# dusk-network/schnorr

Measured on AMD Instinct MI355X. Metric: Schnorr verifies/sec (single + double) at batch=2^20; 1/2/4/8 MI355X, higher is better.
Workload: dtype u32x9 (29-bit limbs, u64 accumulate); 1 GPU; 2^20 single-signature batch verify per GPU (BASELINE configs[1]); `value` is this figure, `double` / `vargen` / `mixed` ride along with --full; batch_per_gpu=1048576, parallelism=dp1, collective=none

## Files before the change

schnorr_amd/csrc/dsv_host.h:

```cpp
#pragma once
#include <hip/hip_runtime.h>

#include <atomic>
#include <chrono>
#include <condition_variable>
#include <cstdarg>
#include <cstdio>
#include <cstring>
#include <functional>
#include <initializer_list>
#include <mutex>
#include <string>
#include <thread>
#include <type_traits>
#include <vector>

#include <errno.h>
#include <sys/random.h>

#include "../../include/dsv.h"
#include "launch.h"
#include "rlc.h"
#include "host_sync.h"

namespace dsvh {

using namespace dsv;
typedef uint32_t u32;

extern thread_local std::string g_err;
int fail(int code, const char* fmt, ...);
#define HIP_TRY(expr)                                                                         \
  do {                                                                                        \
    hipError_t e_ = (expr);                                                                   \
    if (e_ != hipSuccess)                                                                     \
      return fail(DSV_ERR_HIP, "%s failed: %s (%s:%d)", #expr, hipGetErrorString(e_), __FILE__, \
                  __LINE__);                                                                  \
  } while (0)

constexpr int kPipeSlots = 8;
constexpr int kMaxDevices = 16;
constexpr int kSplitLanes = 8;

struct SplitLane {
  hipStream_t owner = nullptr;
  bool made = false;
  hipStream_t stream[2] = {nullptr, nullptr};
  hipStream_t side = nullptr;
  hipEvent_t fork = nullptr, join[2] = {nullptr, nullptr}, side_join = nullptr;
};

struct PipeSlot {
  hipEvent_t ev_in = nullptr;
  hipEvent_t ev_pre = nullptr;
  hipEvent_t ev_lane[2] = {nullptr, nullptr};
  hipEvent_t ev_done = nullptr;
  uint8_t* prep = nullptr;
  size_t prep_bytes = 0;
  uint8_t* stage = nullptr;
  size_t bytes = 0;
  uint8_t* host = nullptr;
  size_t host_bytes = 0;
};
struct Pipe {
  PipeSlot slot[kPipeSlots];
  CopyPool copiers;
};

struct Context {
  std::atomic<bool> ready{false};
  int device = -1;
  std::string pci_bdf;
  int numa_node = -1;
  std::vector<int> numa_cpus;
  bool split = true;
  bool fuse_double = true;
  bool quad = true;
  bool small_overlap = true;
  u32* table[2] = {nullptr, nullptr};
  u32* ts_cancel = nullptr;
  uint8_t* ts_hash = nullptr;
  std::mutex mu;
  uint8_t* stage = nullptr;
  size_t stage_bytes = 0;
  std::mutex lane_mu;
  SplitLane lanes[kSplitLanes];
  PipeSync pipe_sync;
  Pipe pipes[kPipes];
  std::mutex enq_mu;
  bool pipe_made = false;
  bool pipe_failed = false;
  hipStream_t pipe_in = nullptr, pipe_out = nullptr, pipe_lane[2] = {nullptr, nullptr}, pipe_pre = nullptr;
  hipStream_t pipe_small = nullptr;
  uint8_t* pipe_work[3] = {};
  size_t pipe_work_bytes[3] = {};
  uint64_t pipe_parts = 0;
  long lane_load[2] = {0, 0};
  bool prep_stream = false;
  PlanParams plan;
  int pipe_slots = 0;
  int norm_per_lane = 0, norm_block = 0;
  struct RlcHostArena {
    std::mutex mu;
    uint8_t* dev = nullptr;
    size_t bytes = 0;
    hipStream_t stream = nullptr;
    hipEvent_t ev[2] = {nullptr, nullptr};
  } rlc_arenas[2];
  std::mutex rlc_pinned_mu;
  u32* rlc_pinned = nullptr;
  std::atomic<u32> rlc_slot{0};
};
extern Context g_ctx[kMaxDevices];
extern std::mutex g_init_mu;
extern std::atomic<int> g_primary;
extern thread_local int t_device;
extern std::mutex g_jobs_mu;
extern std::condition_variable g_jobs_cv;
extern int g_jobs;

struct DeviceGuard {
  int prev = -1;
  bool switched = false;
  hipError_t err = hipSuccess;
  explicit DeviceGuard(int device) {
    err = hipGetDevice(&prev);
    if (err == hipSuccess && prev != device) {
      err = hipSetDevice(device);
      switched = err == hipSuccess;
    }
  }
  ~DeviceGuard() {
    if (switched) (void)hipSetDevice(prev);
  }
};
#define DSV_ON_DEVICE(ctx)                     \
  DeviceGuard guard_((ctx).device);            \
  if (guard_.err != hipSuccess)                \
  return fail(DSV_ERR_HIP, "cannot select device %d: %s", (ctx).device, hipGetErrorString(guard_.err))

int ensure_stage(Context& ctx, size_t bytes);
void destroy_pipe_streams(Context& ctx);
int ensure_pipe_streams(Context& ctx);
int ensure_pipe_work(Context& ctx, int lane, size_t bytes);
int ensure_pipe_slot(PipeSlot& sl, size_t dev_bytes, size_t host_bytes, size_t prep_bytes);
int check_n(size_t n);
int host_context(Context*& out);
int device_context(const void* ptr, Context*& out);
void release_context(Context& ctx);
void keysets_release_device(int device);

struct Workspace {
  uint8_t* c;
  uint8_t* valid;
  u32* tables;
};
constexpr int kTablesPerLane = 3;
inline size_t var_table_bytes(size_t n, int tables_per_lane) {
  return (size_t)verify_grid(n) * kVerifyBlock * kVarLaneWords * 4 * (size_t)tables_per_lane;
}
inline Workspace carve(void* ws, size_t n) {
  Workspace w;
  w.c = static_cast<uint8_t*>(ws);
  w.valid = w.c + align_up(n * 32, 256);
  w.tables = reinterpret_cast<u32*>(w.valid + align_up(n, 256));
  return w;
}

struct Stager {
  uint8_t* base;
  size_t off = 0;
  explicit Stager(uint8_t* b) : base(b) {}
  uint8_t* take(size_t bytes) {
    uint8_t* p = base + off;
    off += align_up(bytes, 256);
    return p;
  }
};

void launch_verify_fixed(const Context& ctx, bool accumulate, const void* u, const void* c,
                         const void* PK_uv, const void* R_uv, int which, const void* valid,
                         size_t n, void* ok, u32* tables, hipStream_t s, bool tables_ready = false,
                         const u32* gate = nullptr);
void launch_verify_fixed_double(const Context& ctx, const void* u, const void* c, const void* PK_uv,
                                const void* R_uv, const void* PKp_uv, const void* Rp_uv,
                                const void* valid, size_t n, void* ok, u32* tables, hipStream_t s,
                                bool tables_ready = false, const u32* gate = nullptr);


int acquire_lane(Context& ctx, hipStream_t user, SplitLane*& out);
template <class Part>
int run_split(Context& ctx, size_t n, void* workspace, hipStream_t user, Part part) {
  Workspace w = carve(workspace, n);
  if (!ctx.split || n < 2 * kSplitItems) {
    part((size_t)0, n, w, user);
    HIP_TRY(hipGetLastError());
    return DSV_OK;
  }
  SplitLane* lane = nullptr;
  if (int r = acquire_lane(ctx, user, lane)) return r;
  std::lock_guard<std::mutex> lk(ctx.lane_mu);
  HIP_TRY(hipEventRecord(lane->fork, user));
  const size_t tbl_words = var_table_bytes(kSplitItems, kTablesPerLane) / 4;
  for (int k = 0; k < 2; k++) HIP_TRY(hipStreamWaitEvent(lane->stream[k], lane->fork, 0));
  size_t off = 0;
  for (size_t p = 0; off < n; p++) {
    const size_t cnt = n - off < kSplitItems ? n - off : kSplitItems;
    const int k = (int)(p & 1);
    Workspace wp;
    wp.c = w.c + off * 32;
    wp.valid = w.valid + off;
    wp.tables = w.tables + (size_t)k * tbl_words;
    part(off, cnt, wp, lane->stream[k]);
    off += cnt;
  }
  HIP_TRY(hipGetLastError());
  for (int k = 0; k < 2; k++) {
    HIP_TRY(hipEventRecord(lane->join[k], lane->stream[k]));
    HIP_TRY(hipStreamWaitEvent(user, lane->join[k], 0));
  }
  return DSV_OK;
}

#define DSV_DEV_PROLOGUE(n, owner_ptr)              \
  if (int r_ = check_n(n)) return r_;               \
  if ((n) == 0) return DSV_OK;                      \
  Context* ctxp_ = nullptr;                         \
  if (int r_ = device_context(owner_ptr, ctxp_)) return r_; \
  Context& ctx = *ctxp_;                            \
  DSV_ON_DEVICE(ctx)


struct SchemeLayout {
  int points;
  size_t sig_bytes, pk_bytes;
  int R, Rp, PK, PKp, Gen;
  bool fixed;
};
constexpr SchemeLayout kSchemes[3] = {
    {2, 64, 32, 0, -1, 1, -1, -1, true},
    {4, 96, 64, 0, 1, 2, 3, -1, true},
    {3, 64, 64, 0, -1, 1, -1, 2, false},
};
inline const SchemeLayout& layout(int scheme) { return kSchemes[scheme]; }
struct Items {
  int scheme = 0;
  const uint8_t* u = nullptr;
  const uint8_t* pt[4] = {};
  const uint8_t* m = nullptr;
  Items at(size_t off, size_t pt_bytes = 64) const {
    Items r = *this;
    r.u = u + 32 * off;
    for (int k = 0; k < layout(scheme).points; k++) r.pt[k] = pt[k] ? pt[k] + pt_bytes * off : nullptr;
    r.m = m ? m + 32 * off : nullptr;
    return r;
  }
  const uint8_t* slot(int k) const { return k < 0 ? nullptr : pt[k]; }
  const uint8_t* R() const { return slot(layout(scheme).R); }
  const uint8_t* Rp() const { return slot(layout(scheme).Rp); }
  const uint8_t* PK() const { return slot(layout(scheme).PK); }
  const uint8_t* PKp() const { return slot(layout(scheme).PKp); }
  const uint8_t* Gen() const { return slot(layout(scheme).Gen); }
  bool any_null() const {
    bool r = !u || !m;
    for (int k = 0; k < layout(scheme).points; k++) r = r || !pt[k];
    return r;
  }
};
inline Items make_items(int scheme, const void* u, std::initializer_list<const void*> pts, const void* m) {
  Items in{scheme, static_cast<const uint8_t*>(u)};
  int k = 0;
  for (const void* p : pts) in.pt[k++] = static_cast<const uint8_t*>(p);
  in.m = static_cast<const uint8_t*>(m);
  return in;
}

extern thread_local bool t_pipeline_part;
extern thread_local size_t t_chunk_first;
void launch_hash(const Items& in, size_t n, uint8_t* c, uint8_t* valid, hipStream_t s, const uint8_t* valid_in = nullptr);
void launch_verify(const Context& ctx, const Items& in, const uint8_t* c, const uint8_t* valid, size_t n,
                   uint8_t* ok, u32* tables, hipStream_t s, bool prebuilt = false, const u32* gate = nullptr);
int verify_on(Context& ctx, const Items& in, size_t n, void* ok, void* workspace, hipStream_t stream,
              const uint8_t* valid_in = nullptr);
void normalize_on(int scheme, const uint8_t* const* in, uint8_t* const* out, size_t n, uint8_t* valid, u32* prefix,
                  hipStream_t s, const uint8_t* u_mont = nullptr, const uint8_t* m_mont = nullptr,
                  uint8_t* u_out = nullptr, uint8_t* m_out = nullptr, int per_lane = 0, int block = 0);
int decompress_on(Context& ctx, const void* in, size_t in_stride, size_t n, void* out_uv, void* ok,
                  int accumulate, hipStream_t stream);

struct RlcStaged {
  ChaChaKey key;
  size_t boundary;
};
int verify_rlc_on(Context& ctx, const Items& in, size_t n, void* ok, void* workspace, hipStream_t s, int window_bits,
                  u32* accepted_dev, bool and_into = false, bool have_challenges = false,
                  const uint8_t* valid_in = nullptr, const RlcStaged* staged = nullptr);
struct RlcVerdictTarget {
  u32* dev = nullptr;
  u32* slot = nullptr;
  int* out = nullptr;
};
int rlc_verdict_target(Context& ctx, int* accepted, RlcVerdictTarget& t);
int rlc_verdict_wait(const RlcVerdictTarget& t, hipStream_t s);
int rlc_clear_accepted(int* accepted);
int rlc_history(Context& ctx);
void carve_rlc_buffers(Stager& st, const RlcPlan& p, RlcBuffers& b);
size_t rlc_group_items(size_t n);
int rlc_split_groups(size_t cnt, int window_bits);
RlcPlan rlc_group_plan(int scheme, size_t cnt, int window_bits, int groups, bool keyed = false);
int check_rlc_bits(int window_bits);
int rlc_random_key(ChaChaKey& key);
int refuse_capture(hipStream_t s, const char* what);
void rlc_plan_words(const RlcPlan& p, size_t bytes, uint64_t* out);
int rlc_forced_groups();
u32* rlc_keyed_history(Context& ctx);

#define H2D(dst, src, bytes) HIP_TRY(hipMemcpyAsync((dst), (src), (bytes), hipMemcpyHostToDevice, 0))
#define D2H(dst, src, bytes) HIP_TRY(hipMemcpyAsync((dst), (src), (bytes), hipMemcpyDeviceToHost, 0))
#define DSV_HOST_PROLOGUE(n)                                  \
  if (int r_ = check_n(n)) return r_;                         \
  if ((n) == 0) return DSV_OK;                                \
  Context* ctxp_ = nullptr;                                   \
  if (int r_ = host_context(ctxp_)) return r_;                \
  Context& ctx = *ctxp_
#define DSV_HOST_LOCK()                                                                \
  std::lock_guard<std::mutex> lk(ctx.mu);                                              \
  if (!ctx.ready.load(std::memory_order_acquire))                                      \
    return fail(DSV_ERR_NOT_INITIALIZED, "device %d was shut down", ctx.device);       \
  DSV_ON_DEVICE(ctx)


constexpr size_t kExtItemBytes = 4 * 64 + 1 + 4 * kLimbs * 4 + 1;
constexpr size_t kMontItemBytes = kExtItemBytes + 64;
enum Form { kAffine, kExt, kMont };
inline size_t form_pt_bytes(int form) { return form == kAffine ? 64 : 96; }
int check_cols(int scheme, const dsv_column* cols, size_t n, const uint8_t* ok, int form);
int verify_host_cols(int scheme, int form, const dsv_column* cols, size_t n, uint8_t* ok, bool multi);

struct WireWs {
  uint8_t *u, *R, *Rp, *P0, *P1, *valid;
  Items items(int scheme, const void* m) const {
    const uint8_t* sig_pts[2] = {R, Rp};
    const uint8_t* pk_pts[2] = {P0, P1};
    const int ns = (int)(layout(scheme).sig_bytes / 32) - 1;
    Items in{scheme, u};
    for (int k = 0; k < layout(scheme).points; k++) in.pt[k] = k < ns ? sig_pts[k] : pk_pts[k - ns];
    in.m = static_cast<const uint8_t*>(m);
    return in;
  }
};
WireWs carve_wire(Stager& x, size_t n);
int decode_wire(Context& ctx, int scheme, const uint8_t* sig, const uint8_t* pk, size_t n, const Items& out,
                uint8_t* valid, hipStream_t st);
int verify_wire(Context& ctx, int scheme, const uint8_t* sig, const uint8_t* pk, const uint8_t* m,
                size_t n, uint8_t* ok);

}
```

schnorr_amd/csrc/k_verify.hip:

```cpp
#include "common.h"
#include "halfgcd.h"

namespace dsv {

template <int NCHAIN>
__global__ void __launch_bounds__(kVerifyBlock, kWavesVerify)
k_verify_fixed_half(const uint8_t* __restrict__ u, const uint8_t* __restrict__ c, ChainOperands op0,
                    ChainOperands op1, const uint8_t* __restrict__ valid, bool accumulate, size_t n,
                    uint8_t* __restrict__ ok, u32* __restrict__ var_tables, const u32* __restrict__ gate) {
  if (gate_says_done(gate)) return;
  u32* tbl = var_tables + ((size_t)blockIdx.x * kVerifyBlock + threadIdx.x) * kJointLaneWords;
#pragma unroll 1
  for (size_t base = (size_t)blockIdx.x * kVerifyBlock; base < n;
       base += (size_t)gridDim.x * kVerifyBlock) {
    const size_t i = base + threadIdx.x;
    if (i >= n) continue;
    bool good = accumulate ? (ok[i] != 0) : (valid[i] != 0);
    u32 ya[8], yb[8], w[8];
    bool b_neg;
    int top;
    {
      u32 cs[8], a[8], b[8];
      load_words8(cs, c, i);
      half_scalars(a, b, b_neg, cs);
      recode_signed2(ya, a);
      recode_signed2(yb, b);
      u32 nz[8];
#pragma unroll
      for (int k = 0; k < 8; k++) nz[k] = (ya[k] ^ 0x55555555u) | (yb[k] ^ 0x55555555u);
      top = top_digit2(nz);
      u32 us[8];
      load_words8(us, u, i);
      const bool u_ok = words_lt(us, kR32);
      good &= u_ok;
      if (!u_ok) us[7] &= 0x0fffffffu;
      fr_mul(w, b, us);
      if (b_neg) {
        const u32 zero[8] = {0, 0, 0, 0, 0, 0, 0, 0};
        u32 t[8];
        fr_sub(t, zero, w);
#pragma unroll
        for (int k = 0; k < 8; k++) w[k] = t[k];
      }
    }
#pragma unroll 1
    for (int h = 0; h < NCHAIN; h++) {
      const ChainOperands op = h ? op1 : op0;
      {
        Fe pku, pkv, ru, rv;
        good &= load_fq(pku, op.PK_uv, 2 * i);
        good &= load_fq(pkv, op.PK_uv, 2 * i + 1);
        good &= load_fq_signed(ru, op.R_uv, 2 * i, !b_neg);
        good &= load_fq(rv, op.R_uv, 2 * i + 1);
        build_joint_table(tbl, pku, pkv, ru, rv);
      }
      Ext acc = ext_from_niels(load_var_entry(tbl, joint_digit(ya, yb, top)));
      {
        RawNiels e = load_var_entry_raw(tbl, joint_digit(ya, yb, top > 0 ? top - 1 : 0));
#pragma unroll 1
        for (int k = top - 1; k >= 0; k--) {
          acc = ext_mul4(acc);
          const Niels cur = finish_var_entry(e);
          e = load_var_entry_raw(tbl, joint_digit(ya, yb, k > 0 ? k - 1 : 0));
          acc = ext_add_niels(acc, cur);
        }
      }
      good &= fixed_base_accumulate_is_identity(acc, w, op.table);
    }
    ok[i] = good ? 1 : 0;
  }
}

void launch_verify_half(int nchain, bool accumulate, const uint8_t* u, const uint8_t* c,
                        ChainOperands op0, ChainOperands op1, const uint8_t* valid, size_t n,
                        uint8_t* ok, uint32_t* var_tables, hipStream_t s, const uint32_t* gate) {
  const dim3 grid(verify_grid(n)), block(kVerifyBlock);
  if (nchain == 2)
    hipLaunchKernelGGL(k_verify_fixed_half<2>, grid, block, 0, s, u, c, op0, op1, valid, accumulate, n,
                       ok, var_tables, gate);
  else
    hipLaunchKernelGGL(k_verify_fixed_half<1>, grid, block, 0, s, u, c, op0, op1, valid, accumulate, n,
                       ok, var_tables, gate);
}

}
```

schnorr_amd/csrc/launch.h:

```cpp
#pragma once
#include <hip/hip_runtime.h>
#include <stddef.h>
#include <stdint.h>

namespace dsv {

constexpr int kLimbs = 9;

constexpr int kFixedBits = 16;
constexpr int kFixedWindows = (253 + kFixedBits - 1) / kFixedBits;
constexpr int kFixedEntries = (1 << (kFixedBits - 1)) + 1;
constexpr int kEntryWords = 4 * kLimbs;
constexpr size_t kTableBytes = (size_t)kFixedWindows * kFixedEntries * kEntryWords * 4;
static_assert(kFixedWindows * kFixedBits <= 288 && kFixedBits >= 4 && kFixedBits <= 16, "window");

constexpr int kVarEntries = 9;
constexpr int kVarEntryWords = 4 * kLimbs;
constexpr int kVarLaneWords = kVarEntries * kVarEntryWords;
constexpr int kVerifyBlock = 64;
constexpr unsigned kMaxVerifyGrid = 4096;
constexpr int kWavesVerify = 2, kWavesHash = 2;

constexpr int kQuadBlock = 256;
constexpr size_t kQuadMaxItems = (size_t)1 << 14;
constexpr size_t kVarHexMaxItems = (size_t)1 << 13;

constexpr int kSplitThreads = 256;
constexpr int kSplitPerThread = 16;
constexpr int kSplitTile = kSplitThreads * kSplitPerThread;

inline unsigned grid_for(size_t n, unsigned block = 256) { return (unsigned)((n + block - 1) / block); }
inline unsigned verify_grid(size_t n) {
  const unsigned g = grid_for(n, kVerifyBlock);
  return g < kMaxVerifyGrid ? g : kMaxVerifyGrid;
}

struct ChainOperands {
  const uint8_t* PK_uv;
  const uint8_t* R_uv;
  const uint32_t* table;
};
struct ChaChaKey {
  uint32_t w[8];
};

hipError_t hash_upload_constants();
void launch_challenge(bool dbl, const uint8_t* R_uv, const uint8_t* Rp_uv, const uint8_t* m, size_t n,
                      uint8_t* c, uint8_t* valid, hipStream_t s, const uint8_t* valid_in = nullptr);
inline __device__ bool gate_says_done(const uint32_t* gate) { return gate && gate[0] == 0u && gate[1] == 1u; }
void launch_verify_half(int nchain, bool accumulate, const uint8_t* u, const uint8_t* c,
                        ChainOperands op0, ChainOperands op1, const uint8_t* valid, size_t n,
                        uint8_t* ok, uint32_t* var_tables, hipStream_t s, const uint32_t* gate = nullptr);
void launch_verify_half_quad(int nchain, bool accumulate, bool tables_ready, const uint8_t* u,
                             const uint8_t* c, ChainOperands op0, ChainOperands op1,
                             const uint8_t* valid, size_t n, uint8_t* ok, uint32_t* var_tables,
                             hipStream_t s, const uint32_t* gate = nullptr);
void launch_prep_var_tables(const uint8_t* PK_uv, const uint8_t* R_uv, size_t n, uint32_t* var_tables,
                            hipStream_t s);
void launch_verify_var(const uint8_t* u, const uint8_t* c, const uint8_t* PK_uv, const uint8_t* Gen_uv,
                       const uint8_t* R_uv, const uint8_t* valid, size_t n, uint8_t* ok,
                       uint32_t* var_tables, hipStream_t s, const uint32_t* gate = nullptr);
void launch_debug_lattice3(const uint8_t* u, const uint8_t* c, size_t n, uint8_t* out, hipStream_t s);
void launch_debug_half_scalars(const uint8_t* c, size_t n, uint8_t* out, hipStream_t s);
void launch_var_base_points(const uint8_t* scalar, const uint8_t* P_uv, size_t n, uint8_t* out_uv,
                            uint32_t* var_tables, hipStream_t s);
void launch_build_fixed_table(uint32_t* table, int which, hipStream_t s);
void launch_fixed_base_points(const uint8_t* scalar, const uint32_t* table, size_t n, uint8_t* out_uv,
                              hipStream_t s);
struct NormalizeArgs {
  const uint8_t* in[4];
  uint8_t* out[4];
  const uint8_t* u_mont = nullptr;
  const uint8_t* m_mont = nullptr;
  uint8_t* u_out = nullptr;
  uint8_t* m_out = nullptr;
};
constexpr int kNormalizePerLane = 32;
inline size_t normalize_lanes(size_t n, int& per_lane, int want_per_lane = 0) {
  per_lane = n >= ((size_t)1 << 19) ? 16 : (n >= ((size_t)1 << 15) ? 8 : 1);
  if (want_per_lane > 0) per_lane = want_per_lane > kNormalizePerLane ? kNormalizePerLane : want_per_lane;
  return (n + per_lane - 1) / per_lane;
}
inline size_t normalize_prefix_bytes(size_t n, int npoints) {
  return (size_t)npoints * (n + kNormalizePerLane) * kLimbs * 4;
}
void launch_normalize_uvz(const NormalizeArgs& a, int npoints, size_t n, uint8_t* valid,
                          uint32_t* prefix, hipStream_t s, int want_per_lane = 0, int block = 0);
void launch_sign_finish(const uint8_t* r, const uint8_t* c, const uint8_t* sk, size_t n, uint8_t* u_out,
                        hipStream_t s);
void launch_decompress(const uint8_t* in, size_t in_stride, size_t n, uint8_t* out_uv, uint8_t* ok,
                       int accumulate, const uint32_t* ts_cancel, const uint8_t* ts_hash, hipStream_t s);
void launch_gather32(const uint8_t* in, size_t stride, size_t n, uint8_t* out, hipStream_t s);
void launch_stdrng_triples(ChaChaKey key, size_t first_item, size_t n, uint8_t* sk, uint8_t* m,
                           uint8_t* r, hipStream_t s);
void launch_stdrng_quads(ChaChaKey key, size_t first_item, size_t n, uint8_t* sk, uint8_t* g,
                         uint8_t* m, uint8_t* r, hipStream_t s);
void launch_debug_fq_mul(const uint8_t* a, const uint8_t* b, size_t n, uint8_t* out, hipStream_t s);
void launch_split_kinds(const uint8_t* kinds, size_t n, uint32_t* tile_counts, uint32_t* totals,
                        uint32_t* idx0, size_t cap0, uint32_t* idx1, size_t cap1, hipStream_t s);
void launch_gather_rows(const void* src, size_t src_rows, uint32_t row16, const uint32_t* idx,
                        size_t count, const uint32_t* limit, void* dst, hipStream_t s);
void launch_scatter_bytes(const uint8_t* src, const uint32_t* idx, size_t count, const uint32_t* limit,
                          uint8_t* dst, size_t dst_len, hipStream_t s);
void launch_mixed_check(const uint32_t* totals, uint32_t want0, uint32_t want1, uint8_t* ok, size_t n,
                        hipStream_t s);

}
```

Baseline: 85.98 million verifies/s.

## Sort verify lanes by top joint digit within larger blocks to cut divergence

The block grows to a configurable group of 256 threads. Each item's top recoded digit is computed first, then items are counting-sorted in shared memory by that digit, so lanes in a wave run similar ladder lengths and divergence in the variable-base loop drops. Item index, sign and top digit are packed into a meta word, and the scalar words are exchanged through LDS. This adds shared-memory traffic, three block barriers per iteration and a larger block under the same launch bounds, which could cost registers or occupancy. The var table sizing is updated to match the new grid.

```diff
diff --git a/schnorr_amd/csrc/dsv_host.h b/schnorr_amd/csrc/dsv_host.h
--- a/schnorr_amd/csrc/dsv_host.h
+++ b/schnorr_amd/csrc/dsv_host.h
@@ -157,7 +157,7 @@
 };
 constexpr int kTablesPerLane = 3;
 inline size_t var_table_bytes(size_t n, int tables_per_lane) {
-  return (size_t)verify_grid(n) * kVerifyBlock * kVarLaneWords * 4 * (size_t)tables_per_lane;
+  return (size_t)verify_group_grid(n) * kVerifyGroup * kVarLaneWords * 4 * (size_t)tables_per_lane;
 }
 inline Workspace carve(void* ws, size_t n) {
   Workspace w;
diff --git a/schnorr_amd/csrc/k_verify.hip b/schnorr_amd/csrc/k_verify.hip
--- a/schnorr_amd/csrc/k_verify.hip
+++ b/schnorr_amd/csrc/k_verify.hip
@@ -3,39 +3,80 @@
 
 namespace dsv {
 
+constexpr int kXchgWords = 14;
+constexpr int kXchgKeys = 129;
+
 template <int NCHAIN>
-__global__ void __launch_bounds__(kVerifyBlock, kWavesVerify)
+__global__ void __launch_bounds__(kVerifyGroup, kWavesVerify)
 k_verify_fixed_half(const uint8_t* __restrict__ u, const uint8_t* __restrict__ c, ChainOperands op0,
                     ChainOperands op1, const uint8_t* __restrict__ valid, bool accumulate, size_t n,
                     uint8_t* __restrict__ ok, u32* __restrict__ var_tables, const u32* __restrict__ gate) {
   if (gate_says_done(gate)) return;
-  u32* tbl = var_tables + ((size_t)blockIdx.x * kVerifyBlock + threadIdx.x) * kJointLaneWords;
+  constexpr int G = kVerifyGroup;
+  __shared__ u32 xchg[kXchgWords * G];
+  constexpr int kHistRounds = (kXchgKeys + G - 1) / G;
+  __shared__ u32 hist[kHistRounds * G];
+  u32* tbl = var_tables + ((size_t)blockIdx.x * G + threadIdx.x) * kJointLaneWords;
 #pragma unroll 1
-  for (size_t base = (size_t)blockIdx.x * kVerifyBlock; base < n;
-       base += (size_t)gridDim.x * kVerifyBlock) {
-    const size_t i = base + threadIdx.x;
-    if (i >= n) continue;
-    bool good = accumulate ? (ok[i] != 0) : (valid[i] != 0);
-    u32 ya[8], yb[8], w[8];
-    bool b_neg;
-    int top;
+  for (size_t base = (size_t)blockIdx.x * G; base < n; base += (size_t)gridDim.x * G) {
+    u32 tid = threadIdx.x;
+    asm volatile("" : "+v"(tid));
+#pragma unroll
+    for (int e = 0; e < kHistRounds; e++) hist[e * G + tid] = 0;
+    u32 ya[8], b[8];
+    u32 key = 0, meta = tid << 9;
+    if (base + tid < n) {
+      u32 cs[8], nz[8];
+      bool b_neg;
+      load_words8(cs, c, base + tid);
+      {
+        u32 a[8], yb[8];
+        half_scalars(a, b, b_neg, cs);
+        recode_signed2(ya, a);
+        recode_signed2(yb, b);
+#pragma unroll
+        for (int k = 0; k < 8; k++) nz[k] = (ya[k] ^ 0x55555555u) | (yb[k] ^ 0x55555555u);
+      }
+      key = (u32)top_digit2(nz) + 1;
+      meta |= key | (b_neg ? 0x100u : 0u);
+    }
+    __syncthreads();
+    u32 rank = atomicAdd(&hist[key], 1u);
+    __syncthreads();
+#pragma unroll 1
+    for (u32 k = 0; k < key; k++) rank += hist[k];
+    if (key != 0) {
+#pragma unroll
+      for (int k = 0; k < 8; k++) xchg[k * G + rank] = ya[k];
+#pragma unroll
+      for (int k = 0; k < 5; k++) xchg[(8 + k) * G + rank] = b[k];
+    }
+    xchg[13 * G + rank] = meta;
+    __syncthreads();
+    meta = xchg[13 * G + tid];
+    if ((meta & 0xffu) == 0) continue;
+    auto unpack = [&meta]() {
+      u32 m = meta;
+      asm volatile("" : "+v"(m));
+      return m;
+    };
+    const auto item = [&]() { return base + (unpack() >> 9); };
+    const auto sign = [&]() { return (unpack() & 0x100u) != 0; };
+#pragma unroll
+    for (int k = 0; k < 8; k++) ya[k] = xchg[k * G + tid];
+#pragma unroll
+    for (int k = 0; k < 8; k++) b[k] = k < 5 ? xchg[(8 + k) * G + tid] : 0u;
+    bool good = true;
+    u32 yb[8], w[8];
     {
-      u32 cs[8], a[8], b[8];
-      load_words8(cs, c, i);
-      half_scalars(a, b, b_neg, cs);
-      recode_signed2(ya, a);
       recode_signed2(yb, b);
-      u32 nz[8];
-#pragma unroll
-      for (int k = 0; k < 8; k++) nz[k] = (ya[k] ^ 0x55555555u) | (yb[k] ^ 0x55555555u);
-      top = top_digit2(nz);
       u32 us[8];
-      load_words8(us, u, i);
+      load_words8(us, u, item());
       const bool u_ok = words_lt(us, kR32);
       good &= u_ok;
       if (!u_ok) us[7] &= 0x0fffffffu;
       fr_mul(w, b, us);
-      if (b_neg) {
+      if (sign()) {
         const u32 zero[8] = {0, 0, 0, 0, 0, 0, 0, 0};
         u32 t[8];
         fr_sub(t, zero, w);
@@ -46,7 +87,10 @@
 #pragma unroll 1
     for (int h = 0; h < NCHAIN; h++) {
       const ChainOperands op = h ? op1 : op0;
+      const int top = (int)(unpack() & 0xffu) - 1;
       {
+        const size_t i = item();
+        const bool b_neg = sign();
         Fe pku, pkv, ru, rv;
         good &= load_fq(pku, op.PK_uv, 2 * i);
         good &= load_fq(pkv, op.PK_uv, 2 * i + 1);
@@ -67,6 +111,8 @@
       }
       good &= fixed_base_accumulate_is_identity(acc, w, op.table);
     }
+    const size_t i = item();
+    good &= accumulate ? (ok[i] != 0) : (valid[i] != 0);
     ok[i] = good ? 1 : 0;
   }
 }
@@ -74,7 +120,7 @@
 void launch_verify_half(int nchain, bool accumulate, const uint8_t* u, const uint8_t* c,
                         ChainOperands op0, ChainOperands op1, const uint8_t* valid, size_t n,
                         uint8_t* ok, uint32_t* var_tables, hipStream_t s, const uint32_t* gate) {
-  const dim3 grid(verify_grid(n)), block(kVerifyBlock);
+  const dim3 grid(verify_group_grid(n)), block(kVerifyGroup);
   if (nchain == 2)
     hipLaunchKernelGGL(k_verify_fixed_half<2>, grid, block, 0, s, u, c, op0, op1, valid, accumulate, n,
                        ok, var_tables, gate);
diff --git a/schnorr_amd/csrc/launch.h b/schnorr_amd/csrc/launch.h
--- a/schnorr_amd/csrc/launch.h
+++ b/schnorr_amd/csrc/launch.h
@@ -19,6 +19,11 @@
 constexpr int kVarLaneWords = kVarEntries * kVarEntryWords;
 constexpr int kVerifyBlock = 64;
 constexpr unsigned kMaxVerifyGrid = 4096;
+#ifndef DSV_VERIFY_GROUP
+#define DSV_VERIFY_GROUP 256
+#endif
+constexpr int kVerifyGroup = DSV_VERIFY_GROUP;
+static_assert(kVerifyGroup == 128 || kVerifyGroup == 256 || kVerifyGroup == 512, "whole waves, keys fit the zeroing loop");
 constexpr int kWavesVerify = 2, kWavesHash = 2;
 
 constexpr int kQuadBlock = 256;
@@ -33,6 +38,9 @@
 inline unsigned verify_grid(size_t n) {
   const unsigned g = grid_for(n, kVerifyBlock);
   return g < kMaxVerifyGrid ? g : kMaxVerifyGrid;
+}
+inline unsigned verify_group_grid(size_t n) {
+  return (verify_grid(n) * (unsigned)kVerifyBlock + kVerifyGroup - 1) / kVerifyGroup;
 }
 
 struct ChainOperands {
```

New measurement: 85.66 million verifies/s. No clear change (-0.4%).
